# ryantd/tf-operator

Measured on AMD Instinct MI355X. Metric: samples/sec (1-worker TFJob), higher is better.
Workload: dtype bf16

## Files before the change

### csrc/asm/gemm_gen.py

```python
#!/usr/bin/env python3
from __future__ import annotations

import sys

LINE = 1056
HALF = 32 * LINE
STAGE = 2 * HALF
LDS_BYTES = 2 * STAGE
KARG_BYTES = 96

KARG = {
    "X": 0, "W": 8, "C": 16, "S": 24,
    "ldx": 32, "ldw": 36, "ldc": 40, "lds": 44,
    "ktiles": 48, "tiles_m": 52, "tiles_n": 56, "xq": 60, "xr": 64,
    "per_group": 68, "fw": 72, "fc": 76, "map": 80, "grid": 84, "phase": 88, "m": 92,
}
MAP_WALK_COLS = 16
MAP_DEFAULT = 2

EPIS = ("plain", "swiglu_fwd", "swiglu_bwd", "rope", "delta", "resadd")

S_ARGS = 4
S_X, S_W, S_C, S_S = 4, 6, 8, 10
S_LDX, S_LDW, S_LDC, S_LDS = 12, 13, 14, 15
# ... 1846 lines not shown
        parts.append(body)
        metas.append(meta)
    for vname, knobs in SWIGLU_BWD_VARIANTS:
        body, meta = _with_knobs(knobs, lambda: kernel("swiglu_bwd", variant=vname))
        parts.append(body)
        metas.append(meta)
    for epi, vname, knobs in SWIGLU_PERSIST_VARIANTS:
        body, meta = _with_knobs(knobs, lambda: kernel(epi, variant=vname))
        parts.append(body)
        metas.append(meta)
    import attn_gen
    import wgrad_gen

    def wgrad_round4():
        saved = dict(wgrad_gen.KNOBS)
        wgrad_gen.KNOBS.update(map="spread", zero_late=False)
        try:
            return wgrad_gen.kernel("v1")
        finally:
            wgrad_gen.KNOBS.clear()
            wgrad_gen.KNOBS.update(saved)

    import attn_bwd_gen

    for body, meta in (wgrad_gen.kernel(), wgrad_round4(), *attn_gen.all_kernels(), probe_kernel(), kernel("plain", trace=True),
                       _with_knobs({"timing": 1}, lambda: kernel("plain", variant="timing")),
                       _with_knobs({"timing": 2}, lambda: kernel("plain", variant="timing2")),
                       *attn_bwd_gen.all_kernels(),
                       *(kernel_nn(epi) for epi in NN_EPIS)):
        parts.append(body)
        metas.append(meta)
    parts.append(".text\n.p2alignl 6, 3212836864\n.fill 256, 4, 3212836864")
    parts.append(".amdgpu_metadata\n---\namdhsa.version:\n  - 1\n  - 2\namdhsa.target: amdgcn-amd-amdhsa--gfx950\namdhsa.kernels:\n" + "".join(metas)
                 + "...\n.end_amdgpu_metadata")
    return "\n".join(parts) + "\n"


if __name__ == "__main__":
    out = sys.argv[1] if len(sys.argv) > 1 else "gemm_tn_asm.s"
    with open(out, "w") as f:
        f.write(generate())
```

### csrc/hip/attention.hip

```cpp
#include <cstdlib>
#include <cstring>

#include "toa_common.h"

typedef __attribute__((ext_vector_type(8))) short bf16x8;
typedef __attribute__((ext_vector_type(4))) short bf16x4;
typedef __attribute__((ext_vector_type(16))) float f32x16;

#define LOG2E 1.4426950408889634f
#define EXP2(x) __builtin_amdgcn_exp2f(x)
#define RESCALE_THR 8.0f

__device__ __forceinline__ f32x16 mfma32(bf16x8 a, bf16x8 b, f32x16 c) {
  return __builtin_amdgcn_mfma_f32_32x32x16_bf16(a, b, c, 0, 0, 0);
}

__device__ __forceinline__ bf16x8 as_bf16x8(u32x4 v) { return __builtin_bit_cast(bf16x8, v); }

#define TK 64
template <int D>
struct AG {
  static constexpr int NCH = D / 8;
  static constexpr int ROWB = 2 * D;
  static constexpr int NS = D / 16;
// ... 1437 lines not shown
    const char* e = getenv("TOA_ATTN_DKDV");
    return !(e && strcmp(e, "hip") == 0);
  }();
  return g_dkdv_variant == 1 || (g_dkdv_variant < 0 && env_on);
}

template <int D, bool ROPE>
static void dkdv_ds_launch(hipStream_t stream, const bf16_t* q, const bf16_t* k, const bf16_t* v, const bf16_t* dout,
                           const float* nlse2, const float* delta, bf16_t* dk, bf16_t* dv, bf16_t* ds, int B, int H,
                           int Hk, int S, float scale, int o_bshd, const float* cosv, const float* sinv, int H3) {
  if (D == 128 && !g_attn_tstat && attn_dkdv_asm_on()) {
    if (toa_attn_dkdv_asm(q, k, v, dout, nlse2, delta, dk, dv, ds, B, H, Hk, S, D, scale, o_bshd | (ROPE ? 2 : 0),
                          cosv, sinv, H3, stream) == 0)
      return;
  }
  const dim3 grid((S / 128) * B * Hk), block(512);
  if (g_attn_tstat)
    hipLaunchKernelGGL((attn_bwd_dkdv_ds_kernel<D, ROPE, true>), grid, block, 0, stream, q, k, v, dout, nlse2, delta,
                       dk, dv, ds, B, H, Hk, S, scale, scale * LOG2E, o_bshd, cosv, sinv, H3, g_attn_tstat);
  else
    hipLaunchKernelGGL((attn_bwd_dkdv_ds_kernel<D, ROPE>), grid, block, 0, stream, q, k, v, dout, nlse2, delta, dk,
                       dv, ds, B, H, Hk, S, scale, scale * LOG2E, o_bshd, cosv, sinv, H3, nullptr);
}
static bool attn_bwd_uses_ds(int S) { return attn_bwd_variant() >= 1 && S % FWD_QB == 0; }
static int64_t attn_ds_blocks_bytes(int B, int H, int S) {
  const int64_t nb = S / 32;
  return (int64_t)B * H * (nb * (nb + 1) / 2) * 2048;
}
static int64_t attn_ds_bytes(int B, int H, int S) {
  return attn_ds_blocks_bytes(B, H, S) + (int64_t)B * H * S * 4 + 2048;
}
extern "C" int64_t toa_attn_bwd_ws_bytes(int B, int H, int S, int D) {
  (void)D;
  return attn_bwd_uses_ds(S) ? attn_ds_bytes(B, H, S) : 0;
}

template <int D, bool TAIL>
static void attn_set_lds_limits() {
  static bool done = false;
  if (done) return;
  (void)hipFuncSetAttribute((const void*)attn_fwd_kernel<D, TAIL>, hipFuncAttributeMaxDynamicSharedMemorySize,
                            4 * AG<D>::TILEB);
  (void)hipFuncSetAttribute((const void*)attn_bwd_dkdv_kernel<D, TAIL>, hipFuncAttributeMaxDynamicSharedMemorySize,
                            DKV<D>::LDS);
  (void)hipFuncSetAttribute((const void*)attn_bwd_dq_kernel<D, TAIL>, hipFuncAttributeMaxDynamicSharedMemorySize,
                            4 * AG<D>::TILEB);
// ... 20 lines not shown
      return (int)hipGetLastError();
    }
  }
  hipLaunchKernelGGL((attn_fwd_kernel<D, TAIL>), dim3(nqb * H * B), dim3(64 * FWD_WAVES), 4 * AG<D>::TILEB, stream, q, k, v,
                     o, lse, B, H, Hk, S, scale * LOG2E, o_bshd);
  return (int)hipGetLastError();
}

template <int D, bool TAIL>
static int attn_bwd_launch(const bf16_t* q, const bf16_t* k, const bf16_t* v, const bf16_t* o, const bf16_t* dout,
                           const float* lse, float* delta, void* ws, bf16_t* dq, bf16_t* dk, bf16_t* dv, int B, int H,
                           int Hk, int S, int o_bshd, float scale, hipStream_t stream) {
  attn_set_lds_limits<D, TAIL>();
  if constexpr (!TAIL) {
    if (attn_bwd_uses_ds(S)) {
      if (ws == nullptr) return (int)hipErrorInvalidValue;
      bf16_t* ds = (bf16_t*)ws;
      float* nlse2 = (float*)((char*)ws + attn_ds_blocks_bytes(B, H, S));
      const int rows = B * H * S;
      hipLaunchKernelGGL((attn_delta_kernel<D>), dim3((rows + 256 / (D / 8) - 1) / (256 / (D / 8))), dim3(256), 0,
                         stream, o, dout, lse, delta, nlse2, rows, H, S, o_bshd);
      dkdv_ds_launch<D, false>(stream, q, k, v, dout, nlse2, delta, dk, dv, ds, B, H, Hk, S, scale, o_bshd, nullptr,
                               nullptr, 0);
      hipLaunchKernelGGL((attn_bwd_dqg_kernel<D>), dim3((S / FWD_QB) * H * B), dim3(512), 0, stream, k, ds, dq, B, H,
                         Hk, S, scale, nullptr, nullptr, 0);
      return (int)hipGetLastError();
    }
  }
  hipLaunchKernelGGL((attn_bwd_dq_kernel<D, TAIL>), dim3(((S + FWD_QB - 1) / FWD_QB) * H * B), dim3(64 * FWD_WAVES),
                     4 * AG<D>::TILEB, stream, q, k, v, dout, o, lse, delta, dq, B, H, Hk, S, scale, scale * LOG2E,
                     o_bshd);
  hipLaunchKernelGGL((attn_bwd_dkdv_kernel<D, TAIL>), dim3(((S + 127) / 128) * B * Hk), dim3(512), DKV<D>::LDS, stream,
                     q, k, v, dout, lse, delta, dk, dv, B, H, Hk, S, scale, scale * LOG2E, o_bshd);
  return (int)hipGetLastError();
}

static bool attn_shape_ok(int B, int H, int Hk, int S, int D, int flags) {
  return (D == 64 || D == 128) && B > 0 && S > 0 && Hk > 0 && H % Hk == 0 && (flags & 1);
}

extern "C" int toa_attn_fwd_asm(const bf16_t* q, const bf16_t* k, const bf16_t* v, bf16_t* o, float* lse, int B,
                                int H, int Hk, int S, int D, int flags, float scale, hipStream_t stream);
static bool attn_fwd_asm_on() {
  static const bool env_on = [] {
    const char* e = getenv("TOA_ATTN_FWD");
    return !(e && strcmp(e, "hip") == 0);
  }();
  return g_fwd_variant == 2 || (g_fwd_variant < 0 && env_on);
// ... 44 lines not shown
}

extern "C" int toa_attn_bwd_rope(const bf16_t* q, const bf16_t* k, const bf16_t* v, const bf16_t* o,
                                 const bf16_t* dout, const float* lse, float* delta, void* ws, const float* cosv,
                                 const float* sinv, bf16_t* dqkv, int B, int H, int Hk, int S, int D, int flags,
                                 float scale, hipStream_t stream) {
  if (!attn_shape_ok(B, H, Hk, S, D, flags)) return (int)hipErrorInvalidValue;
  if (!attn_bwd_uses_ds(S)) return (int)hipErrorNotSupported;
  if (ws == nullptr || dqkv == nullptr || cosv == nullptr || sinv == nullptr) return (int)hipErrorInvalidValue;
  const int o_bshd = (flags >> 1) & 1;
  const int H3 = H + 2 * Hk;
  bf16_t* ds = (bf16_t*)ws;
  float* nlse2 = (float*)((char*)ws + attn_ds_blocks_bytes(B, H, S));
  const int rows = B * H * S;
#define TOA_ATTN_BWD_ROPE(DD)                                                                                    \
  do {                                                                                                           \
    if (flags & 4)                                                                                               \
      hipLaunchKernelGGL(attn_nlse2_kernel, dim3((rows + 255) / 256), dim3(256), 0, stream, lse, nlse2, rows);   \
    else                                                                                                         \
      hipLaunchKernelGGL((attn_delta_kernel<DD>), dim3((rows + 256 / (DD / 8) - 1) / (256 / (DD / 8))),          \
                         dim3(256), 0, stream, o, dout, lse, delta, nlse2, rows, H, S, o_bshd);                  \
    dkdv_ds_launch<DD, true>(stream, q, k, v, dout, nlse2, delta, dqkv, dqkv, ds, B, H, Hk, S, scale, o_bshd,  \
                             cosv, sinv, H3);                                                                   \
    hipLaunchKernelGGL((attn_bwd_dqg_kernel<DD, true>), dim3((S / FWD_QB) * H * B), dim3(512), 0, stream, k, ds, \
                       dqkv, B, H, Hk, S, scale, cosv, sinv, H3);                                               \
  } while (0)
#ifdef TOA_ATTN_D128_ONLY
  if (D != 128) return (int)hipErrorInvalidValue;
  TOA_ATTN_BWD_ROPE(128);
#else
  if (D == 128)
    TOA_ATTN_BWD_ROPE(128);
  else
    TOA_ATTN_BWD_ROPE(64);
#endif
#undef TOA_ATTN_BWD_ROPE
  return (int)hipGetLastError();
}
```

### csrc/hip/gemm_asm.hip

```cpp
#include <hip/hip_runtime.h>

#include <cstdint>
#include <cstdlib>
#include <cstring>
#include <mutex>

#include "toa_common.h"

namespace {

#include "toa_asm_blob.inc"

constexpr int kMaxDev = 64;
enum { K_PLAIN = 0, K_SWIGLU_FWD = 1, K_SWIGLU_BWD = 2, K_PROBE = 3, K_TRACE = 4, K_TIMING = 5, K_TIMING2 = 6,
       K_WGRAD = 7, K_V1 = 8, K_WGRAD_V1 = 16, K_ATTN_FWD = 17, K_ATTN_D1 = 18, K_ATTN_T1 = 23,
       K_ATTN_DKDV = 26, K_DKDV_D1 = 27, K_DKDV_T1 = 34, K_SWIGLU_FWD_R4 = 41, K_SWIGLU_BWD_R4 = 42, K_SWBWD_V1 = 43, K_PLAIN_V9 = 48, K_DKDV_S7 = 49, K_DKDV_D8 = 50, K_DKDV_S8 = 51, K_SWFWD_P1 = 52, K_SWBWD_P1 = 53, K_ROPE = 54, K_DELTA = 55, K_RESADD = 56, K_N = 57 };
const char* kNames[K_N] = {"toa_gemm_tn_asm_plain",    "toa_gemm_tn_asm_swiglu_fwd", "toa_gemm_tn_asm_swiglu_bwd",
                           "toa_gemm_tn_asm_probe",    "toa_gemm_tn_asm_trace",      "toa_gemm_tn_asm_timing",
                           "toa_gemm_tn_asm_timing2",  "toa_wgrad_nt_asm",           "toa_gemm_tn_asm_plain_v1",
                           "toa_gemm_tn_asm_plain_v2", "toa_gemm_tn_asm_plain_v3", "toa_gemm_tn_asm_plain_v4",
                           "toa_gemm_tn_asm_plain_v5", "toa_gemm_tn_asm_plain_v6", "toa_gemm_tn_asm_plain_v7",
                           "toa_gemm_tn_asm_plain_v8", "toa_wgrad_nt_asm_v1",       "toa_attn_fwd_asm",
                           "toa_attn_fwd_asm_d1",      "toa_attn_fwd_asm_d2",        "toa_attn_fwd_asm_d3",
                           "toa_attn_fwd_asm_d4",      "toa_attn_fwd_asm_d5",        "toa_attn_fwd_asm_t1",
                           "toa_attn_fwd_asm_c1",      "toa_attn_fwd_asm_t2",        "toa_attn_dkdv_asm",
                           "toa_attn_dkdv_asm_d1",     "toa_attn_dkdv_asm_d2",       "toa_attn_dkdv_asm_d3",
                           "toa_attn_dkdv_asm_d4",     "toa_attn_dkdv_asm_d5",       "toa_attn_dkdv_asm_d6",
                           "toa_attn_dkdv_asm_d7",     "toa_attn_dkdv_asm_t1",
                           "toa_attn_dkdv_asm_s1",     "toa_attn_dkdv_asm_s2",       "toa_attn_dkdv_asm_s3",
                           "toa_attn_dkdv_asm_s4",     "toa_attn_dkdv_asm_s5",       "toa_attn_dkdv_asm_s6",
                           "toa_gemm_tn_asm_swiglu_fwd_r4", "toa_gemm_tn_asm_swiglu_bwd_r4",
                           "toa_gemm_tn_asm_swiglu_bwd_b1", "toa_gemm_tn_asm_swiglu_bwd_b2",
                           "toa_gemm_tn_asm_swiglu_bwd_b3", "toa_gemm_tn_asm_swiglu_bwd_b4",
                           "toa_gemm_tn_asm_swiglu_bwd_b5",
                           "toa_gemm_tn_asm_plain_v9",
                           "toa_attn_dkdv_asm_s7", "toa_attn_dkdv_asm_d8", "toa_attn_dkdv_asm_s8",
                           "toa_gemm_tn_asm_swiglu_fwd_p1", "toa_gemm_tn_asm_swiglu_bwd_p1",
                           "toa_gemm_tn_asm_rope",
                           "toa_gemm_tn_asm_delta",
                           "toa_gemm_tn_asm_resadd"};

enum { NN_PLAIN = 0, NN_SWIGLU_BWD = 1, NN_DELTA = 2, NN_N = 3 };
const char* kNnNames[NN_N] = {"toa_gemm_nn_asm_plain", "toa_gemm_nn_asm_swiglu_bwd", "toa_gemm_nn_asm_delta"};

constexpr int kNnBase = 1 << 16;

struct DevModule {
  std::once_flag once;
  hipError_t err = hipSuccess;
  hipModule_t mod = nullptr;
  hipFunction_t fn[K_N] = {};
  hipFunction_t nn[NN_N] = {};
};
DevModule g_mod[kMaxDev];

hipFunction_t get_fn(int which, hipError_t* err) {
  int dev = 0;
  if ((*err = hipGetDevice(&dev)) != hipSuccess) return nullptr;
  if (dev < 0 || dev >= kMaxDev) {
    *err = hipErrorInvalidDevice;
    return nullptr;
  }
  DevModule& m = g_mod[dev];
  std::call_once(m.once, [&m]() {
    m.err = hipModuleLoadData(&m.mod, toa_asm_blob);
    for (int i = 0; m.err == hipSuccess && i < K_N; ++i) m.err = hipModuleGetFunction(&m.fn[i], m.mod, kNames[i]);
    for (int i = 0; m.err == hipSuccess && i < NN_N; ++i) m.err = hipModuleGetFunction(&m.nn[i], m.mod, kNnNames[i]);
  });
  *err = m.err;
  return m.err == hipSuccess ? (which >= kNnBase ? m.nn[which - kNnBase] : m.fn[which]) : nullptr;
}

struct __attribute__((packed)) Args {
  uint64_t X, W, C, S;
  uint32_t ldx, ldw, ldc, lds;
  uint32_t ktiles, tiles_m, tiles_n, xq, xr, per_group;
  uint32_t fw, fc;
  uint32_t map;
  uint32_t grid;
  uint32_t phase;
  uint32_t m;
};
static_assert(sizeof(Args) == 96, "kernarg block must match csrc/asm/gemm_gen.py KARG_BYTES");

constexpr uint32_t kMapDefault = 2;
constexpr uint32_t kMapWalkCols = 16;

bool ld_ok(int64_t ld, int64_t min_cols) { return ld >= min_cols && ld % 8 == 0 && ld * 2 * 256 < (1ll << 32); }
bool al16(const void* p) { return ((uintptr_t)p & 15) == 0; }

constexpr int kNumPlainVariants = 9;
constexpr int kVariantFn[kNumPlainVariants] = {K_V1,     K_V1 + 1, K_V1 + 2, K_V1 + 3,  K_V1 + 4,
                                               K_V1 + 5, K_V1 + 6, K_V1 + 7, K_PLAIN_V9};
// ... 612 lines not shown
  a.dout = (uint64_t)dout;
  a.nlse2 = (uint64_t)nlse2;
  a.ndelta = (uint64_t)ndelta;
  a.dk = (uint64_t)dk;
  a.dv = (uint64_t)dv;
  a.ds = (uint64_t)ds;
  a.cosv = (uint64_t)cosv;
  a.sinv = (uint64_t)sinv;
  a.B = (uint32_t)B;
  a.H = (uint32_t)H;
  a.Hk = (uint32_t)Hk;
  a.S = (uint32_t)S;
  a.scale = scale;
  a.c = scale * 1.4426950408889634f;
  a.flags = (uint32_t)flags;
  a.rep = (uint32_t)(H / Hk);
  a.nkb = (uint32_t)(S / 128);
  a.H3 = (uint32_t)(rope ? H3 : 0);
  a.dbg = (uint64_t)dbg;
  size_t sz = sizeof(a);
  void* cfg[] = {HIP_LAUNCH_PARAM_BUFFER_POINTER, &a, HIP_LAUNCH_PARAM_BUFFER_SIZE, &sz, HIP_LAUNCH_PARAM_END};
  return (int)hipModuleLaunchKernel(fn, (unsigned)nwg, 1, 1, 256, 1, 1, 0, stream, nullptr, cfg);
}
```

### tf_operator_amd/ops/_lib.py

```python
from __future__ import annotations

import ctypes
import os
import threading

import torch

_HERE = os.path.dirname(os.path.abspath(__file__))
LIB_PATH = os.environ.get("TOA_HIP_LIB") or os.path.join(os.path.dirname(_HERE), "lib", "libtoa_hip.so")

_lock = threading.Lock()
_lib = None
_err = None

c_int = ctypes.c_int
c_i64 = ctypes.c_int64
c_f = ctypes.c_float
c_p = ctypes.c_void_p

_SIGS = {
    "toa_sumsq": [c_p, c_i64, c_int, c_p, c_p, c_int, c_p],
    "toa_adamw_flat": [c_p, c_p, c_p, c_int, c_p, c_p, c_i64, c_f, c_f, c_f, c_f, c_f, c_int, c_f, c_p, c_f, c_p],
    "toa_adamw_flat_dstep": [c_p, c_p, c_p, c_int, c_p, c_p, c_i64, c_f, c_f, c_f, c_f, c_f, c_p, c_f, c_p, c_f,
                             c_p],
# ... 74 lines not shown
    "toa_gemm_asm_rows": [c_p, c_i64, c_p, c_i64, c_p, c_i64, c_int, c_int, c_int, c_p],
    "toa_gemm_asm_swiglu": [c_p, c_i64, c_p, c_i64, c_p, c_i64, c_p, c_i64, c_int, c_int, c_int, c_p],
    "toa_gemm_asm_swiglu_bwd": [c_p, c_i64, c_p, c_i64, c_p, c_i64, c_p, c_i64, c_int, c_int, c_int, c_p],
    "toa_gemm_asm_swiglu_bwd_variant": [c_int, c_p, c_i64, c_p, c_i64, c_p, c_i64, c_p, c_i64, c_int, c_int, c_int, c_p],
    "toa_gemm_asm_available": [],
    "toa_gemm_asm_trace": [c_p, c_p, c_i64, c_p, c_i64, c_p, c_i64, c_int, c_int, c_int, c_p],
    "toa_host_free": [c_p],
    "toa_gemm_asm_stage": [c_int, c_p, c_i64, c_p, c_i64, c_p, c_i64, c_int, c_int, c_int, c_p],
    "toa_gemm_asm_variant": [c_int, c_p, c_i64, c_p, c_i64, c_p, c_i64, c_int, c_int, c_int, c_p],
    "toa_gemm_asm_map": [c_int, c_p, c_i64, c_p, c_i64, c_p, c_i64, c_int, c_int, c_int, c_p],
    "toa_gemm_asm_set_epi_variant": [c_int],
    "toa_gemm_asm_set_phase": [c_int, ctypes.c_uint],
    "toa_wgrad_asm_set_map": [c_int],
    "toa_gemm_asm_set_map": [c_int],
    "toa_gemm_asm_set_persist": [c_int],
    "toa_attn_dkdv_asm_set_arm": [c_int],
    "toa_gemm_asm_timing": [c_int, c_p, c_p, c_i64, c_p, c_i64, c_p, c_i64, c_int, c_int, c_int, c_p],
    "toa_gemm_asm_probe": [c_p, c_p, c_i64, c_p, c_i64, c_p, c_i64, c_int, c_int, c_int, c_p],
    "toa_attn_set_bwd_variant": [c_int],
    "toa_attn_set_bwd_timing": [c_p],
    "toa_norm_set_row": [c_int],
    "toa_attn_set_fwd_variant": [c_int],
    "toa_attn_set_dkdv_variant": [c_int],
    "toa_attn_dkdv_asm": [c_p, c_p, c_p, c_p, c_p, c_p, c_p, c_p, c_p, c_int, c_int, c_int, c_int, c_int, c_f, c_int,
                          c_p, c_p, c_int, c_p],
    "toa_attn_dkdv_asm_variant": [c_int, c_p, c_p, c_p, c_p, c_p, c_p, c_p, c_p, c_p, c_int, c_int, c_int, c_int, c_int,
                                  c_f, c_int, c_p, c_p, c_int, c_p],
    "toa_attn_dkdv_asm_timing": [c_p, c_p, c_p, c_p, c_p, c_p, c_p, c_p, c_p, c_p, c_int, c_int, c_int, c_int, c_int,
                                 c_f, c_int, c_p, c_p, c_int, c_p],
    "toa_attn_bwd_rope": [c_p, c_p, c_p, c_p, c_p, c_p, c_p, c_p, c_p, c_p, c_p, c_int, c_int, c_int, c_int, c_int,
                          c_int, c_f, c_p],
    "toa_emulate_xfer": [c_p, c_p, c_i64, c_int, ctypes.c_double, c_p],
    "toa_emulate_copy_nocu": [c_p, c_p, c_i64, c_p],
    "toa_flag_publish": [c_p, ctypes.c_uint, c_p],
    "toa_flags_wait": [c_p, c_int, c_int, c_int, ctypes.c_uint, c_p, c_int, c_p],
    "toa_copy_nocu": [c_p, c_p, c_i64, c_p],
    "toa_sum_slices_bf16": [c_p, c_p, c_int, c_i64, c_i64, c_p],
    "toa_gemm_tune": [c_int, c_int, c_i64, c_i64, c_i64, c_p, c_i64, c_p, c_i64, c_p, c_i64, c_f, c_int, c_p, c_p, c_p,
                      c_p, c_p, c_int],
    "toa_gemm_kernel_name": [c_int, c_int, c_i64, c_i64, c_i64, c_i64, c_i64, c_i64, c_int, c_int, c_p, c_int],
}


def _load():
    global _lib, _err
    with _lock:
# ... 101 lines not shown
```

Baseline: 6.583.

## Add hand-written assembly kernel for attention backward dQ from stored dS

```diff
diff --git a/csrc/asm/attn_dq_gen.py b/csrc/asm/attn_dq_gen.py
--- /dev/null
+++ b/csrc/asm/attn_dq_gen.py
@@ -0,0 +1,508 @@
+#!/usr/bin/env python3
+from __future__ import annotations
+
+import sys
+
+import attn_gen as AG
+import gemm_gen as G
+from attn_gen import Item, schedule
+from gemm_gen import Asm, ar, sr, vr
+
+NAME = "toa_attn_dq_asm"
+D = 128
+ROWB = 2 * D
+TK = 64
+KT = TK * ROWB
+DSB = 2048
+DSW = 4 * DSB
+SLOT = KT + 4 * DSW
+NSLOT = 3
+LDS_BYTES = NSLOT * SLOT
+RING = 6
+LEAD = 4
+DL_DMA = 10
+KARG_BYTES = 80
+KARG = {"K": 0, "dS": 8, "dQ": 16, "cos": 24, "sin": 32, "B": 40, "H": 44, "Hk": 48, "S": 52, "scale": 56,
+        "flags": 60, "nqb": 64, "rep": 68, "g8": 72, "H3": 76}
+
+S_K, S_DS, S_DQP, S_COS, S_SIN = 4, 6, 8, 10, 12
+S_B, S_H, S_HK, S_S, S_SC, S_FL = 14, 15, 16, 17, 18, 19
+S_NQB, S_REP, S_G8, S_H3 = 20, 21, 22, 23
+S_W, S_QB, S_HH, S_BB, S_HKV = 24, 25, 26, 27, 28
+S_T, S_TW, S_TL = 29, 30, 31
+S_CUR, S_NX, S_IT, S_NXK, S_NXD, S_KSO, S_DSA0, S_DSA1 = 32, 33, 34, 35, 36, 37, 38, 39
+SRD_K, SRD_DS, SRD_O, SRD_C, SRD_S = 40, 44, 48, 52, 56
+S_T0 = AG.S_T0
+S_DQ, S_DR = AG.S_DQ, AG.S_DR
+S_TRI0, S_TRI1, S_KM0, S_DM0, S_Q0, S_OSTR, S_SOFF, S_OJ = 70, 71, 72, 73, 74, 75, 76, 77
+N_SGPR = 96
+assert (S_T0, S_DQ, S_DR) == (60, 68, 69)
+
+V_TRO, V_TRO8, V_DSO = 1, 5, 9
+V_CTRO, V_CTRO8, V_CDSO = 13, 17, 21
+V_T = 24
+V_KD = 32
+V_DSG = 36
+V_KF = 40
+V_SF = 64
+V_CS, V_SN = 96, 160
+V_X = 224
+A_ACC = 0
+
+
+def kf(f):
+    return V_KF + 4 * (f % RING)
+
+
+def sfreg(j, n, s2):
+    return V_SF + 4 * (4 * j + 2 * n + s2)
+
+
+def k_piece(u: int) -> list[str]:
+    return [f"s_add_u32 m0, {sr(S_NXK)}, {1024 * u}",
+            "s_nop 0",
+            f"buffer_load_dwordx4 {vr(V_KD + u)}, {sr(SRD_K, 4)}, {sr(S_KSO)} offen lds"]
+
+
+def ds_piece(j: int, n: int, half: int) -> list[str]:
+    base = S_DSA0 if j == 0 else S_DSA1
+    out = [f"s_add_u32 {sr(S_SOFF)}, {sr(base)}, {DSB}"] if n else []
+    so = S_SOFF if n else base
+    return out + [f"s_add_u32 m0, {sr(S_NXD)}, {2 * DSB * j + DSB * n + 1024 * half}",
+                  "s_nop 0",
+                  f"buffer_load_dwordx4 {vr(V_DSG + half)}, {sr(SRD_DS, 4)}, {sr(so)} offen nt lds"]
+
+
+def dma_setup() -> list[str]:
+    return [f"s_lshl_b32 {sr(S_KSO)}, {sr(S_IT)}, 14",
+            f"s_add_u32 {sr(S_NXK)}, {sr(S_NX)}, {sr(S_KM0)}",
+            f"s_lshl_b32 {sr(S_T0)}, {sr(S_IT)}, 12",
+            f"s_add_u32 {sr(S_DSA0)}, {sr(S_TRI0)}, {sr(S_T0)}",
+            f"s_add_u32 {sr(S_DSA1)}, {sr(S_TRI1)}, {sr(S_T0)}",
+            f"s_add_u32 {sr(S_NXD)}, {sr(S_NX)}, {sr(S_DM0)}"]
+
+
+N_FULL, N_DIAG, N_KONLY = 12, 10, 4
+
+
+def issue_generic(a: Asm):
+    skip, nods = a.fresh("iss_done"), a.fresh("iss_no01")
+    a(f"s_cmp_gt_u32 {sr(S_IT)}, {sr(S_TL)}")
+    a(f"s_cbranch_scc1 {skip}")
+    for x in dma_setup():
+        a(x)
+    for u in range(4):
+        for x in k_piece(u):
+            a(x)
+    a(f"s_cmp_gt_u32 {sr(S_IT)}, {sr(S_TW)}")
+    a(f"s_cbranch_scc1 {skip}")
+    for half in range(2):
+        for x in ds_piece(0, 0, half):
+            a(x)
+    a(f"s_cmp_eq_u32 {sr(S_IT)}, {sr(S_TW)}")
+    a(f"s_cbranch_scc1 {nods}")
+    for half in range(2):
+        for x in ds_piece(0, 1, half):
+            a(x)
+    a.label(nods)
+    for n in range(2):
+        for half in range(2):
+            for x in ds_piece(1, n, half):
+                a(x)
+    a.label(skip)
+
+
+def tile_mfmas(diag: bool) -> list:
+    out = []
+    for n in range(2):
+        for s2 in range(2):
+            for dt in range(4):
+                f = 8 * n + 4 * s2 + dt
+                for j in range(2):
+                    if diag and n == 1 and j == 0:
+                        continue
+                    acc = ar(A_ACC + 64 * j + 16 * dt, 16)
+                    out.append((f"v_mfma_f32_32x32x16_bf16 {acc}, {vr(kf(f), 4)}, {vr(sfreg(j, n, s2), 4)}, {acc}",
+                                [f"KF{f}", f"SF{j}{n}{s2}"]))
+    return out
+
+
+def kt_read(f: int) -> list[str]:
+    n, r = divmod(f, 8)
+    s2, dt = divmod(r, 4)
+    rb = (32 * n + 16 * s2) * ROWB
+    return [f"ds_read_b64_tr_b16 {vr(kf(f), 2)}, {vr(V_CTRO + dt)} offset:{rb} ; KF{f}",
+            f"ds_read_b64_tr_b16 {vr(kf(f) + 2, 2)}, {vr(V_CTRO8 + dt)} offset:{rb} ; KF{f}"]
+
+
+def ds_read(j: int, n: int, s2: int) -> list[str]:
+    off = 2 * DSB * j + DSB * n
+    return [f"ds_read_b64_tr_b16 {vr(sfreg(j, n, s2), 2)}, {vr(V_CDSO + 2 * s2)} offset:{off} ; SF{j}{n}{s2}",
+            f"ds_read_b64_tr_b16 {vr(sfreg(j, n, s2) + 2, 2)}, {vr(V_CDSO + 2 * s2 + 1)} offset:{off} ; SF{j}{n}{s2}"]
+
+
+def slot_offsets(a: Asm):
+    for i in range(4):
+        a(f"v_add_u32 {vr(V_CTRO + i)}, {sr(S_CUR)}, {vr(V_TRO + i)}")
+        a(f"v_add_u32 {vr(V_CTRO8 + i)}, {sr(S_CUR)}, {vr(V_TRO8 + i)}")
+        a(f"v_add_u32 {vr(V_CDSO + i)}, {sr(S_CUR)}, {vr(V_DSO + i)}")
+
+
+def compute(a: Asm, diag: bool, dma: bool, tail: list | None = None):
+    mf = tile_mfmas(diag)
+    first: dict = {}
+    last: dict = {}
+    for g, (_, tags) in enumerate(mf):
+        for t in tags:
+            first.setdefault(t, g)
+            last[t] = g
+    items: list[Item] = []
+    for f in range(16):
+        rel = -1 if f < RING else last[f"KF{f - RING}"]
+        items.append(Item(kt_read(f), 8, rel, max(rel, first[f"KF{f}"] - LEAD), "kr"))
+    for n in range(2):
+        for s2 in range(2):
+            for j in range(2):
+                if diag and n == 1 and j == 0:
+                    continue
+                items.append(Item(ds_read(j, n, s2), 8, -1, max(-1, first[f"SF{j}{n}{s2}"] - LEAD), "sr"))
+    if dma:
+        for u in range(4):
+            items.append(Item(k_piece(u), 48, -1, DL_DMA, "dma", split=False))
+        for j in range(2):
+            for n in range(2):
+                for half in range(2):
+                    items.append(Item(ds_piece(j, n, half), 48, -1, DL_DMA, "dma", split=False))
+    slot_offsets(a)
+    schedule(a, mf, items, tail)
+
+
+def coords(a: Asm):
+    t0, t1 = S_T0, S_T0 + 1
+    a(f"s_cmp_eq_u32 {sr(S_NQB)}, 0")
+    a(f"s_cbranch_scc1 {a.abort}")
+    a(f"s_lshl_b32 {sr(t0)}, {sr(S_NQB)}, 8")
+    a(f"s_cmp_lg_u32 {sr(t0)}, {sr(S_S)}")
+    a(f"s_cbranch_scc1 {a.abort}")
+    a(f"s_mul_i32 {sr(t0)}, {sr(S_REP)}, {sr(S_HK)}")
+    a(f"s_cmp_lg_u32 {sr(t0)}, {sr(S_H)}")
+    a(f"s_cbranch_scc1 {a.abort}")
+    a(f"s_mul_i32 {sr(t0)}, {sr(S_NQB)}, {sr(S_H)}")
+    a(f"s_mul_i32 {sr(t0)}, {sr(t0)}, {sr(S_B)}")
+    a(f"s_cmp_ge_u32 s2, {sr(t0)}")
+    a(f"s_cbranch_scc1 {a.abort}")
+    a(f"s_mul_i32 {sr(t1)}, {sr(S_B)}, {sr(S_HK)}")
+    lgen, lcoord = a.fresh("coords_generic"), a.fresh("coords_done")
+    a(f"s_cmp_eq_u32 {sr(S_G8)}, 0")
+    a(f"s_cbranch_scc1 {lgen}")
+    a(f"s_and_b32 {sr(t0 + 2)}, {sr(t1)}, 7")
+    a(f"s_cmp_lg_u32 {sr(t0 + 2)}, 0")
+    a(f"s_cbranch_scc1 {a.abort}")
+    a(f"s_and_b32 {sr(S_T0 + 2)}, s2, 7")
+    a(f"s_lshr_b32 {sr(S_T0 + 3)}, s2, 3")
+    a(f"s_lshr_b32 {sr(S_T0 + 4)}, {sr(t1)}, 3")
+    a(f"s_mul_i32 {sr(S_T0 + 5)}, {sr(S_T0 + 4)}, {sr(S_REP)}")
+    AG.udiv(a, S_DQ, S_DR, S_T0 + 3, S_T0 + 5)
+    a(f"s_sub_u32 {sr(S_QB)}, {sr(S_NQB)}, 1")
+    a(f"s_sub_u32 {sr(S_QB)}, {sr(S_QB)}, {sr(S_DQ)}")
+    a(f"s_mov_b32 {sr(S_T0 + 3)}, {sr(S_DR)}")
+    AG.udiv(a, S_DQ, S_DR, S_T0 + 3, S_REP)
+    a(f"s_mul_i32 {sr(S_T0 + 2)}, {sr(S_T0 + 2)}, {sr(S_T0 + 4)}")
+    a(f"s_add_u32 {sr(S_T0 + 2)}, {sr(S_T0 + 2)}, {sr(S_DQ)}")
+    a(f"s_mov_b32 {sr(S_T0 + 5)}, {sr(S_DR)}")
+    AG.udiv(a, S_DQ, S_DR, S_T0 + 2, S_HK)
+    a(f"s_mov_b32 {sr(S_BB)}, {sr(S_DQ)}")
+    a(f"s_mul_i32 {sr(S_HH)}, {sr(S_DR)}, {sr(S_REP)}")
+    a(f"s_add_u32 {sr(S_HH)}, {sr(S_HH)}, {sr(S_T0 + 5)}")
+    a(f"s_branch {lcoord}")
+    a.label(lgen)
+    a(f"s_mul_i32 {sr(S_T0 + 2)}, {sr(S_H)}, {sr(S_B)}")
+    AG.udiv(a, S_DQ, S_DR, 2, S_T0 + 2)
+    a(f"s_sub_u32 {sr(S_QB)}, {sr(S_NQB)}, 1")
+    a(f"s_sub_u32 {sr(S_QB)}, {sr(S_QB)}, {sr(S_DQ)}")
+    a(f"s_mov_b32 {sr(S_T0 + 3)}, {sr(S_DR)}")
+    AG.udiv(a, S_DQ, S_DR, S_T0 + 3, S_H)
+    a(f"s_mov_b32 {sr(S_BB)}, {sr(S_DQ)}")
+    a(f"s_mov_b32 {sr(S_HH)}, {sr(S_DR)}")
+    a.label(lcoord)
+    AG.udiv(a, S_DQ, S_DR, S_HH, S_REP)
+    a(f"s_mov_b32 {sr(S_HKV)}, {sr(S_DQ)}")
+
+
+def prologue(a: Asm):
+    a(f"s_load_dwordx16 {sr(4, 16)}, s[0:1], 0x0")
+    a(f"s_load_dwordx4 {sr(20, 4)}, s[0:1], 0x40")
+    a(f"v_lshrrev_b32 {vr(V_X + 15)}, 6, v0")
+    a("s_waitcnt lgkmcnt(0)")
+    coords(a)
+    t0, t1, t2 = S_T0, S_T0 + 1, S_T0 + 2
+    a("s_nop 4")
+    a(f"v_readfirstlane_b32 {sr(S_W)}, {vr(V_X + 15)}")
+    a("s_nop 4")
+    a(f"s_lshl_b32 {sr(t0)}, {sr(S_QB)}, 2")
+    a(f"s_add_u32 {sr(S_TL)}, {sr(t0)}, 3")
+    a(f"s_add_u32 {sr(S_TW)}, {sr(t0)}, {sr(S_W)}")
+    a(f"s_lshl_b32 {sr(S_Q0)}, {sr(S_QB)}, 8")
+    a(f"s_lshl_b32 {sr(t0)}, {sr(S_W)}, 6")
+    a(f"s_add_u32 {sr(S_Q0)}, {sr(S_Q0)}, {sr(t0)}")
+    a(f"s_lshl_b32 {sr(t0)}, {sr(S_TW)}, 1")
+    a(f"s_add_u32 {sr(t1)}, {sr(t0)}, 1")
+    a(f"s_mul_i32 {sr(t0)}, {sr(t0)}, {sr(t1)}")
+    a(f"s_lshr_b32 {sr(t0)}, {sr(t0)}, 1")
+    a(f"s_lshl_b32 {sr(S_TRI0)}, {sr(t0)}, 11")
+    a(f"s_lshl_b32 {sr(t1)}, {sr(t1)}, 11")
+    a(f"s_add_u32 {sr(S_TRI1)}, {sr(S_TRI0)}, {sr(t1)}")
+    a(f"s_lshl_b32 {sr(S_KM0)}, {sr(S_W)}, 12")
+    a(f"s_lshl_b32 {sr(S_DM0)}, {sr(S_W)}, 13")
+    a(f"s_add_u32 {sr(S_DM0)}, {sr(S_DM0)}, {KT}")
+    a(f"s_mul_i32 {sr(t1)}, {sr(S_BB)}, {sr(S_HK)}")
+    a(f"s_add_u32 {sr(t1)}, {sr(t1)}, {sr(S_HKV)}")
+    a(f"s_mul_i32 {sr(t1)}, {sr(t1)}, {sr(S_S)}")
+    a(f"s_lshl_b32 {sr(t2)}, {sr(S_S)}, 8")
+    AG.srd64(a, SRD_K, S_K, t1, ROWB, sr(t2))
+    a(f"s_lshr_b32 {sr(t0)}, {sr(S_S)}, 5")
+    a(f"s_add_u32 {sr(t1)}, {sr(t0)}, 1")
+    a(f"s_mul_i32 {sr(t0)}, {sr(t0)}, {sr(t1)}")
+    a(f"s_lshr_b32 {sr(t0)}, {sr(t0)}, 1")
+    a(f"s_lshl_b32 {sr(t2)}, {sr(t0)}, 11")
+    a(f"s_mul_i32 {sr(t1)}, {sr(S_BB)}, {sr(S_H)}")
+    a(f"s_add_u32 {sr(t1)}, {sr(t1)}, {sr(S_HH)}")
+    AG.srd64(a, SRD_DS, S_DS, t1, sr(t2), sr(t2))
+    lrope, lodone = a.fresh("o_rope"), a.fresh("o_done")
+    a(f"s_bitcmp1_b32 {sr(S_FL)}, 0")
+    a(f"s_cbranch_scc1 {lrope}")
+    a(f"s_mul_i32 {sr(t1)}, {sr(t1)}, {sr(S_S)}")
+    a(f"s_add_u32 {sr(t1)}, {sr(t1)}, {sr(S_Q0)}")
+    a(f"s_mov_b32 {sr(S_OSTR)}, {ROWB}")
+    AG.srd64(a, SRD_O, S_DQP, t1, ROWB, 64 * ROWB)
+    a(f"s_branch {lodone}")
+    a.label(lrope)
+    a(f"s_mul_i32 {sr(t1)}, {sr(S_BB)}, {sr(S_S)}")
+    a(f"s_add_u32 {sr(t1)}, {sr(t1)}, {sr(S_Q0)}")
+    a(f"s_mul_i32 {sr(t1)}, {sr(t1)}, {sr(S_H3)}")
+    a(f"s_add_u32 {sr(t1)}, {sr(t1)}, {sr(S_HH)}")
+    a(f"s_lshl_b32 {sr(S_OSTR)}, {sr(S_H3)}, 8")
+    a(f"s_mul_i32 {sr(t2)}, {sr(S_OSTR)}, 63")
+    a(f"s_add_u32 {sr(t2)}, {sr(t2)}, {ROWB}")
+    AG.srd64(a, SRD_O, S_DQP, t1, ROWB, sr(t2))
+    AG.srd64(a, SRD_C, S_COS, S_Q0, 256, 64 * 256)
+    AG.srd64(a, SRD_S, S_SIN, S_Q0, 256, 64 * 256)
+    a.label(lodone)
+    l, g, qq, pp, hh, r, tt = (V_X + i for i in range(7))
+    t = V_T
+    a(f"v_and_b32 {vr(l)}, 63, v0")
+    a(f"v_lshrrev_b32 {vr(g)}, 4, {vr(l)}")
+    a(f"v_bfe_u32 {vr(qq)}, {vr(l)}, 2, 2")
+    a(f"v_and_b32 {vr(pp)}, 3, {vr(l)}")
+    a(f"v_lshrrev_b32 {vr(hh)}, 5, {vr(l)}")
+    a(f"v_and_b32 {vr(r)}, 31, {vr(l)}")
+    a(f"v_lshl_add_u32 {vr(tt)}, {vr(hh)}, 2, {vr(qq)}")
+    a(f"v_lshlrev_b32 {vr(tt)}, 8, {vr(tt)}")
+    a(f"v_and_b32 {vr(t)}, 1, {vr(g)}")
+    a(f"v_lshlrev_b32 {vr(t)}, 1, {vr(t)}")
+    a(f"v_lshrrev_b32 {vr(t + 1)}, 1, {vr(pp)}")
+    a(f"v_add_u32 {vr(t)}, {vr(t)}, {vr(t + 1)}")
+    a(f"v_lshl_add_u32 {vr(t + 1)}, {vr(qq)}, 2, {vr(hh)}")
+    a(f"v_add_u32 {vr(t + 2)}, 2, {vr(t + 1)}")
+    a(f"v_and_b32 {vr(t + 3)}, 1, {vr(pp)}")
+    a(f"v_lshlrev_b32 {vr(t + 3)}, 3, {vr(t + 3)}")
+    a(f"v_add_u32 {vr(t + 6)}, {vr(t + 3)}, {vr(tt)}")
+    for dt in range(4):
+        a(f"v_add_u32 {vr(t + 4)}, {4 * dt}, {vr(t)}")
+        a(f"v_xor_b32 {vr(t + 5)}, {vr(t + 4)}, {vr(t + 1)}")
+        a(f"v_lshl_add_u32 {vr(V_TRO + dt)}, {vr(t + 5)}, 4, {vr(t + 6)}")
+        a(f"v_xor_b32 {vr(t + 5)}, {vr(t + 4)}, {vr(t + 2)}")
+        a(f"v_lshl_add_u32 {vr(V_TRO8 + dt)}, {vr(t + 5)}, 4, {vr(t + 6)}")
+        a(f"v_add_u32 {vr(V_TRO8 + dt)}, {8 * ROWB}, {vr(V_TRO8 + dt)}")
+    a(f"v_lshl_add_u32 {vr(t + 4)}, {vr(t)}, 2, {vr(qq)}")
+    a(f"v_lshl_add_u32 {vr(t + 4)}, {vr(hh)}, 2, {vr(t + 4)}")
+    a(f"v_lshlrev_b32 {vr(t + 5)}, 9, {vr(t)}")
+    a(f"v_add_u32 {vr(t + 5)}, {vr(t + 5)}, {vr(t + 3)}")
+    a(f"v_add_u32 {vr(t + 5)}, {sr(S_DM0)}, {vr(t + 5)}")
+    for s2 in range(2):
+        for e in range(2):
+            a(f"v_add_u32 {vr(t + 7)}, {16 * s2 + 8 * e}, {vr(t + 4)}")
+            a(f"v_and_b32 {vr(t + 7)}, 31, {vr(t + 7)}")
+            a(f"v_lshl_add_u32 {vr(V_DSO + 2 * s2 + e)}, {vr(t + 7)}, 4, {vr(t + 5)}")
+    a(f"v_and_b32 {vr(t)}, 15, {vr(l)}")
+    a(f"v_lshlrev_b32 {vr(t + 1)}, 2, {vr(g)}")
+    a(f"v_xor_b32 {vr(t)}, {vr(t)}, {vr(t + 1)}")
+    a(f"v_lshlrev_b32 {vr(t + 1)}, 8, {vr(g)}")
+    a(f"v_add_u32 {vr(t + 1)}, {sr(S_KM0)}, {vr(t + 1)}")
+    for u in range(4):
+        a(f"v_xor_b32 {vr(t + 2)}, {u}, {vr(t)}")
+        a(f"v_lshl_add_u32 {vr(V_KD + u)}, {vr(t + 2)}, 4, {vr(t + 1)}")
+        a(f"v_add_u32 {vr(V_KD + u)}, {4 * u * ROWB}, {vr(V_KD + u)}")
+    for half in range(2):
+        a(f"v_add_u32 {vr(t)}, {2 * half}, {vr(hh)}")
+        a(f"v_lshlrev_b32 {vr(t + 1)}, 2, {vr(t)}")
+        a(f"v_sub_u32 {vr(t + 1)}, {vr(r)}, {vr(t + 1)}")
+        a(f"v_and_b32 {vr(t + 1)}, 31, {vr(t + 1)}")
+        a(f"v_lshl_add_u32 {vr(t + 1)}, {vr(t)}, 5, {vr(t + 1)}")
+        a(f"v_lshlrev_b32 {vr(V_DSG + half)}, 4, {vr(t + 1)}")
+    lnr = a.fresh("no_rope_rows")
+    a(f"s_bitcmp1_b32 {sr(S_FL)}, 0")
+    a(f"s_cbranch_scc0 {lnr}")
+    a(f"v_lshlrev_b32 {vr(t)}, 8, {vr(r)}")
+    a(f"v_lshl_add_u32 {vr(t)}, {vr(hh)}, 4, {vr(t)}")
+    a(f"s_mov_b32 {sr(S_OJ)}, {32 * 256}")
+    for j in range(2):
+        so = sr(S_OJ) if j else "0"
+        for dt in range(2):
+            for g4 in range(4):
+                o = 128 * dt + 32 * g4
+                a(f"buffer_load_dwordx4 {vr(V_CS + 32 * j + 16 * dt + 4 * g4, 4)}, {vr(t)}, {sr(SRD_C, 4)}, {so} "
+                  f"offen offset:{o}")
+                a(f"buffer_load_dwordx4 {vr(V_SN + 32 * j + 16 * dt + 4 * g4, 4)}, {vr(t)}, {sr(SRD_S, 4)}, {so} "
+                  f"offen offset:{o}")
+    a.label(lnr)
+    for x in range(128):
+        a(f"v_accvgpr_write_b32 {ar(A_ACC + x)}, 0")
+    for tile in range(2):
+        a(f"s_mov_b32 {sr(S_IT)}, {tile}")
+        a(f"s_mov_b32 {sr(S_NX)}, {tile * SLOT}")
+        issue_generic(a)
+    a(f"s_mov_b32 {sr(S_T)}, 0")
+    a(f"s_mov_b32 {sr(S_CUR)}, 0")
+    a(f"s_mov_b32 {sr(S_NX)}, {2 * SLOT}")
+
+
+def store_rows(a: Asm, j: int, scaled: bool):
+    oo = V_X + 2
+    so = sr(S_OJ) if j else "0"
+    for dt in range(4):
+        for k in range(2):
+            tmp, data = V_X + 4, V_X + 12
+            base = A_ACC + 64 * j + 16 * dt + 8 * k
+            for e in range(8):
+                a(f"v_accvgpr_read_b32 {vr(tmp + e)}, {ar(base + e)}")
+            if scaled:
+                for e in range(8):
+                    a(f"v_mul_f32 {vr(tmp + e)}, {sr(S_SC)}, {vr(tmp + e)}")
+            for e in range(4):
+                a(f"v_cvt_pk_bf16_f32 {vr(data + e)}, {vr(tmp + 2 * e)}, {vr(tmp + 2 * e + 1)}")
+            a("s_nop 1")
+            a(f"v_permlane32_swap_b32 {vr(data)}, {vr(data + 2)}")
+            a(f"v_permlane32_swap_b32 {vr(data + 1)}, {vr(data + 3)}")
+            a(f"buffer_store_dwordx4 {vr(data, 4)}, {vr(oo)}, {sr(SRD_O, 4)}, {so} offen offset:{64 * dt + 32 * k}")
+            a("s_nop 1")
+
+
+def epilogue(a: Asm):
+    a("s_waitcnt vmcnt(0)")
+    a("s_nop 7")
+    a("s_nop 7")
+    a("s_nop 7")
+    r, hh, oo = V_X, V_X + 1, V_X + 2
+    a(f"v_and_b32 {vr(r)}, 31, v0")
+    a(f"v_bfe_u32 {vr(hh)}, v0, 5, 1")
+    a(f"v_mul_lo_u32 {vr(oo)}, {vr(r)}, {sr(S_OSTR)}")
+    a(f"v_lshl_add_u32 {vr(oo)}, {vr(hh)}, 4, {vr(oo)}")
+    a(f"s_lshl_b32 {sr(S_OJ)}, {sr(S_OSTR)}, 5")
+    lrope, ldone = a.fresh("epi_rope"), a.fresh("epi_done")
+    a(f"s_bitcmp1_b32 {sr(S_FL)}, 0")
+    a(f"s_cbranch_scc1 {lrope}")
+    for j in range(2):
+        store_rows(a, j, True)
+    a(f"s_branch {ldone}")
+    a.label(lrope)
+    y1, y2, p, q = V_T, V_T + 1, V_T + 2, V_T + 3
+    for j in range(2):
+        for dt in range(2):
+            for i in range(16):
+                a1, a2 = A_ACC + 64 * j + 16 * dt + i, A_ACC + 64 * j + 16 * (dt + 2) + i
+                c, s_ = V_CS + 32 * j + 16 * dt + i, V_SN + 32 * j + 16 * dt + i
+                a(f"v_accvgpr_read_b32 {vr(y1)}, {ar(a1)}")
+                a(f"v_accvgpr_read_b32 {vr(y2)}, {ar(a2)}")
+                a(f"v_mul_f32 {vr(y1)}, {sr(S_SC)}, {vr(y1)}")
+                a(f"v_mul_f32 {vr(y2)}, {sr(S_SC)}, {vr(y2)}")
+                a(f"v_mul_f32 {vr(p)}, {vr(s_)}, {vr(y2)}")
+                a(f"v_mul_f32 {vr(q)}, {vr(s_)}, {vr(y1)}")
+                a(f"v_fma_f32 {vr(p)}, {vr(c)}, {vr(y1)}, {vr(p)}")
+                a(f"v_fma_f32 {vr(q)}, {vr(c)}, {vr(y2)}, -{vr(q)}")
+                a(f"v_accvgpr_write_b32 {ar(a1)}, {vr(p)}")
+                a(f"v_accvgpr_write_b32 {ar(a2)}, {vr(q)}")
+    a("s_nop 1")
+    for j in range(2):
+        store_rows(a, j, False)
+    a.label(ldone)
+
+
+def kernel() -> tuple[str, str]:
+    a = Asm(prefix="dq_")
+    a.raw(f".globl {NAME}")
+    a.raw(".p2align 8")
+    a.raw(f".type {NAME},@function")
+    a.raw(f"{NAME}:")
+    prologue(a)
+    lab = {k: a.fresh(k) for k in ("loop", "steady", "next", "w10", "w4", "w0", "wd", "nocomp", "diag", "epi")}
+    t1, t2 = S_T0 + 1, S_T0 + 2
+    a.label(lab["loop"])
+    a(f"s_add_u32 {sr(S_IT)}, {sr(S_T)}, 2")
+    a(f"s_cmp_lt_u32 {sr(S_IT)}, {sr(S_TW)}")
+    a(f"s_cbranch_scc1 {lab['steady']}")
+    a(f"s_add_u32 {sr(t1)}, {sr(S_T)}, 1")
+    a(f"s_cmp_gt_u32 {sr(t1)}, {sr(S_TL)}")
+    a(f"s_cbranch_scc1 {lab['w0']}")
+    a(f"s_cmp_gt_u32 {sr(t1)}, {sr(S_TW)}")
+    a(f"s_cbranch_scc1 {lab['w4']}")
+    a(f"s_cmp_eq_u32 {sr(t1)}, {sr(S_TW)}")
+    a(f"s_cbranch_scc1 {lab['w10']}")
+    a(f"s_waitcnt vmcnt({N_FULL})")
+    a(f"s_branch {lab['wd']}")
+    a.label(lab["w10"])
+    a(f"s_waitcnt vmcnt({N_DIAG})")
+    a(f"s_branch {lab['wd']}")
+    a.label(lab["w4"])
+    a(f"s_waitcnt vmcnt({N_KONLY})")
+    a(f"s_branch {lab['wd']}")
+    a.label(lab["w0"])
+    a("s_waitcnt vmcnt(0)")
+    a.label(lab["wd"])
+    a("s_barrier")
+    issue_generic(a)
+    a(f"s_cmp_gt_u32 {sr(S_T)}, {sr(S_TW)}")
+    a(f"s_cbranch_scc1 {lab['next']}")
+    a(f"s_cmp_eq_u32 {sr(S_T)}, {sr(S_TW)}")
+    a(f"s_cbranch_scc1 {lab['diag']}")
+    compute(a, False, False, [f"s_branch {lab['next']}"])
+    a.label(lab["diag"])
+    compute(a, True, False, [f"s_branch {lab['next']}"])
+    a.label(lab["steady"])
+    a(f"s_waitcnt vmcnt({N_FULL})")
+    a("s_barrier")
+    for x in dma_setup():
+        a(x)
+    compute(a, False, True)
+    a.label(lab["next"])
+    a(f"s_mov_b32 {sr(S_NX)}, {sr(S_CUR)}")
+    a(f"s_add_u32 {sr(S_CUR)}, {sr(S_CUR)}, {SLOT}")
+    a(f"s_cmp_eq_u32 {sr(S_CUR)}, {NSLOT * SLOT}")
+    a(f"s_cselect_b32 {sr(S_CUR)}, 0, {sr(S_CUR)}")
+    a(f"s_add_u32 {sr(S_T)}, {sr(S_T)}, 1")
+    a(f"s_cmp_gt_u32 {sr(S_T)}, {sr(S_TL)}")
+    a(f"s_cbranch_scc0 {lab['loop']}")
+    epilogue(a)
+    a.label(a.abort)
+    a("s_waitcnt vmcnt(0)")
+    a("s_endpgm")
+    a.raw(f".size {NAME}, .-{NAME}")
+    desc, meta = G._descriptor(NAME, lds_bytes=LDS_BYTES, n_sgpr=N_SGPR, karg_bytes=KARG_BYTES)
+    return "\n".join(a.out) + "\n" + desc, meta
+
+
+def all_kernels() -> list[tuple[str, str]]:
+    return [kernel()]
+
+
+def generate(kernels=None) -> str:
+    kernels = kernels or [kernel()]
+    return "\n".join(['.amdgcn_target "amdgcn-amd-amdhsa--gfx950"', ".amdhsa_code_object_version 5", ".text",
+                      *(b for b, _ in kernels),
+                      ".amdgpu_metadata\n---\namdhsa.version:\n  - 1\n  - 2\namdhsa.target: amdgcn-amd-amdhsa--gfx950\n"
+                      "amdhsa.kernels:\n" + "".join(m for _, m in kernels) + "...\n.end_amdgpu_metadata"]) + "\n"
+
+
+if __name__ == "__main__":
+    with open(sys.argv[1] if len(sys.argv) > 1 else "attn_dq_asm.s", "w") as f:
+        f.write(generate())
diff --git a/csrc/asm/gemm_gen.py b/csrc/asm/gemm_gen.py
--- a/csrc/asm/gemm_gen.py
+++ b/csrc/asm/gemm_gen.py
@@ -1892,12 +1892,14 @@
             wgrad_gen.KNOBS.update(saved)
 
     import attn_bwd_gen
+    import attn_dq_gen
 
     for body, meta in (wgrad_gen.kernel(), wgrad_round4(), *attn_gen.all_kernels(), probe_kernel(), kernel("plain", trace=True),
                        _with_knobs({"timing": 1}, lambda: kernel("plain", variant="timing")),
                        _with_knobs({"timing": 2}, lambda: kernel("plain", variant="timing2")),
                        *attn_bwd_gen.all_kernels(),
-                       *(kernel_nn(epi) for epi in NN_EPIS)):
+                       *(kernel_nn(epi) for epi in NN_EPIS),
+                       *attn_dq_gen.all_kernels()):
         parts.append(body)
         metas.append(meta)
     parts.append(".text\n.p2alignl 6, 3212836864\n.fill 256, 4, 3212836864")
diff --git a/csrc/hip/attention.hip b/csrc/hip/attention.hip
--- a/csrc/hip/attention.hip
+++ b/csrc/hip/attention.hip
@@ -1483,6 +1483,35 @@
     hipLaunchKernelGGL((attn_bwd_dkdv_ds_kernel<D, ROPE>), grid, block, 0, stream, q, k, v, dout, nlse2, delta, dk,
                        dv, ds, B, H, Hk, S, scale, scale * LOG2E, o_bshd, cosv, sinv, H3, nullptr);
 }
+extern "C" int toa_attn_dq_asm(const bf16_t* k, const bf16_t* ds, bf16_t* dq, int B, int H, int Hk, int S, int D,
+                               float scale, int flags, const float* cosv, const float* sinv, int H3,
+                               hipStream_t stream);
+static int g_dq_variant = -1;
+extern "C" int toa_attn_set_dq_variant(int v) {
+  if (v < -1 || v > 1) return (int)hipErrorInvalidValue;
+  g_dq_variant = v;
+  return 0;
+}
+static constexpr bool kAttnDqAsmDefault = true;
+static bool attn_dq_asm_on() {
+  static const bool env_on = [] {
+    const char* e = getenv("TOA_ATTN_DQ");
+    if (e && strcmp(e, "hip") == 0) return false;
+    if (e && strcmp(e, "asm") == 0) return true;
+    return kAttnDqAsmDefault;
+  }();
+  return g_dq_variant == 1 || (g_dq_variant < 0 && env_on);
+}
+
+template <int D, bool ROPE>
+static void dq_ds_launch(hipStream_t stream, const bf16_t* k, const bf16_t* ds, bf16_t* dq, int B, int H, int Hk,
+                         int S, float scale, const float* cosv, const float* sinv, int H3) {
+  if (D == 128 && attn_dq_asm_on()) {
+    if (toa_attn_dq_asm(k, ds, dq, B, H, Hk, S, D, scale, ROPE ? 1 : 0, cosv, sinv, H3, stream) == 0) return;
+  }
+  hipLaunchKernelGGL((attn_bwd_dqg_kernel<D, ROPE>), dim3((S / FWD_QB) * H * B), dim3(512), 0, stream, k, ds, dq, B,
+                     H, Hk, S, scale, cosv, sinv, H3);
+}
 static bool attn_bwd_uses_ds(int S) { return attn_bwd_variant() >= 1 && S % FWD_QB == 0; }
 static int64_t attn_ds_blocks_bytes(int B, int H, int S) {
   const int64_t nb = S / 32;
@@ -1549,8 +1578,7 @@
                          stream, o, dout, lse, delta, nlse2, rows, H, S, o_bshd);
       dkdv_ds_launch<D, false>(stream, q, k, v, dout, nlse2, delta, dk, dv, ds, B, H, Hk, S, scale, o_bshd, nullptr,
                                nullptr, 0);
-      hipLaunchKernelGGL((attn_bwd_dqg_kernel<D>), dim3((S / FWD_QB) * H * B), dim3(512), 0, stream, k, ds, dq, B, H,
-                         Hk, S, scale, nullptr, nullptr, 0);
+      dq_ds_launch<D, false>(stream, k, ds, dq, B, H, Hk, S, scale, nullptr, nullptr, 0);
       return (int)hipGetLastError();
     }
   }
@@ -1641,8 +1669,7 @@
                          dim3(256), 0, stream, o, dout, lse, delta, nlse2, rows, H, S, o_bshd);                  \
     dkdv_ds_launch<DD, true>(stream, q, k, v, dout, nlse2, delta, dqkv, dqkv, ds, B, H, Hk, S, scale, o_bshd,  \
                              cosv, sinv, H3);                                                                   \
-    hipLaunchKernelGGL((attn_bwd_dqg_kernel<DD, true>), dim3((S / FWD_QB) * H * B), dim3(512), 0, stream, k, ds, \
-                       dqkv, B, H, Hk, S, scale, cosv, sinv, H3);                                               \
+    dq_ds_launch<DD, true>(stream, k, ds, dqkv, B, H, Hk, S, scale, cosv, sinv, H3);                            \
   } while (0)
 #ifdef TOA_ATTN_D128_ONLY
   if (D != 128) return (int)hipErrorInvalidValue;
diff --git a/csrc/hip/gemm_asm.hip b/csrc/hip/gemm_asm.hip
--- a/csrc/hip/gemm_asm.hip
+++ b/csrc/hip/gemm_asm.hip
@@ -45,12 +45,17 @@
 
 constexpr int kNnBase = 1 << 16;
 
+enum { DQ_ATTN = 0, DQ_N = 1 };
+const char* kDqNames[DQ_N] = {"toa_attn_dq_asm"};
+constexpr int kDqBase = 2 << 16;
+
 struct DevModule {
   std::once_flag once;
   hipError_t err = hipSuccess;
   hipModule_t mod = nullptr;
   hipFunction_t fn[K_N] = {};
   hipFunction_t nn[NN_N] = {};
+  hipFunction_t dq[DQ_N] = {};
 };
 DevModule g_mod[kMaxDev];
 
@@ -66,9 +71,12 @@
     m.err = hipModuleLoadData(&m.mod, toa_asm_blob);
     for (int i = 0; m.err == hipSuccess && i < K_N; ++i) m.err = hipModuleGetFunction(&m.fn[i], m.mod, kNames[i]);
     for (int i = 0; m.err == hipSuccess && i < NN_N; ++i) m.err = hipModuleGetFunction(&m.nn[i], m.mod, kNnNames[i]);
+    for (int i = 0; m.err == hipSuccess && i < DQ_N; ++i) m.err = hipModuleGetFunction(&m.dq[i], m.mod, kDqNames[i]);
   });
   *err = m.err;
-  return m.err == hipSuccess ? (which >= kNnBase ? m.nn[which - kNnBase] : m.fn[which]) : nullptr;
+  if (m.err != hipSuccess) return nullptr;
+  if (which >= kDqBase) return m.dq[which - kDqBase];
+  return which >= kNnBase ? m.nn[which - kNnBase] : m.fn[which];
 }
 
 struct __attribute__((packed)) Args {
@@ -727,3 +735,49 @@
   void* cfg[] = {HIP_LAUNCH_PARAM_BUFFER_POINTER, &a, HIP_LAUNCH_PARAM_BUFFER_SIZE, &sz, HIP_LAUNCH_PARAM_END};
   return (int)hipModuleLaunchKernel(fn, (unsigned)nwg, 1, 1, 256, 1, 1, 0, stream, nullptr, cfg);
 }
+
+struct __attribute__((packed)) DqArgs {
+  uint64_t k, ds, dq, cosv, sinv;
+  uint32_t B, H, Hk, S;
+  float scale;
+  uint32_t flags, nqb, rep, g8, H3;
+};
+static_assert(sizeof(DqArgs) == 80, "kernarg block must match csrc/asm/attn_dq_gen.py KARG_BYTES");
+
+extern "C" int toa_attn_dq_asm(const bf16_t* k, const bf16_t* ds, bf16_t* dq, int B, int H, int Hk, int S, int D,
+                               float scale, int flags, const float* cosv, const float* sinv, int H3,
+                               hipStream_t stream) {
+  const bool rope = (flags & 1) != 0;
+  if (D != 128 || B <= 0 || H <= 0 || Hk <= 0 || H % Hk || S <= 0 || S % 256 || !al16(k) || !al16(ds) || !al16(dq) ||
+      (flags & ~1) || (rope && (!cosv || !sinv || !al16(cosv) || !al16(sinv) || H3 != H + 2 * Hk)))
+    return (int)hipErrorInvalidValue;
+  const int64_t nb = S / 32, nblk = nb * (nb + 1) / 2;
+  const int64_t nwg = (int64_t)(S / 256) * H * B;
+  if (nwg >= (1 << 24) || nblk * 2048 >= (1ll << 32) || (int64_t)S * 256 >= (1ll << 31) ||
+      (int64_t)B * H * S >= (1ll << 32) || (int64_t)B * S * (rope ? H3 : 1) >= (1ll << 32) ||
+      (int64_t)64 * (rope ? H3 : 1) * 256 >= (1ll << 31))
+    return (int)hipErrorInvalidValue;
+  hipError_t err;
+  hipFunction_t fn = get_fn(kDqBase + DQ_ATTN, &err);
+  if (!fn) return (int)err;
+  DqArgs a;
+  memset(&a, 0, sizeof(a));
+  a.k = (uint64_t)k;
+  a.ds = (uint64_t)ds;
+  a.dq = (uint64_t)dq;
+  a.cosv = (uint64_t)cosv;
+  a.sinv = (uint64_t)sinv;
+  a.B = (uint32_t)B;
+  a.H = (uint32_t)H;
+  a.Hk = (uint32_t)Hk;
+  a.S = (uint32_t)S;
+  a.scale = scale;
+  a.flags = (uint32_t)flags;
+  a.nqb = (uint32_t)(S / 256);
+  a.rep = (uint32_t)(H / Hk);
+  a.g8 = ((int64_t)B * Hk) % 8 == 0 ? 1u : 0u;
+  a.H3 = (uint32_t)(rope ? H3 : 0);
+  size_t sz = sizeof(a);
+  void* cfg[] = {HIP_LAUNCH_PARAM_BUFFER_POINTER, &a, HIP_LAUNCH_PARAM_BUFFER_SIZE, &sz, HIP_LAUNCH_PARAM_END};
+  return (int)hipModuleLaunchKernel(fn, (unsigned)nwg, 1, 1, 256, 1, 1, 0, stream, nullptr, cfg);
+}
diff --git a/tf_operator_amd/ops/_lib.py b/tf_operator_amd/ops/_lib.py
--- a/tf_operator_amd/ops/_lib.py
+++ b/tf_operator_amd/ops/_lib.py
@@ -120,6 +120,8 @@
     "toa_norm_set_row": [c_int],
     "toa_attn_set_fwd_variant": [c_int],
     "toa_attn_set_dkdv_variant": [c_int],
+    "toa_attn_set_dq_variant": [c_int],
+    "toa_attn_dq_asm": [c_p, c_p, c_p, c_int, c_int, c_int, c_int, c_int, c_f, c_int, c_p, c_p, c_int, c_p],
     "toa_attn_dkdv_asm": [c_p, c_p, c_p, c_p, c_p, c_p, c_p, c_p, c_p, c_int, c_int, c_int, c_int, c_int, c_f, c_int,
                           c_p, c_p, c_int, c_p],
     "toa_attn_dkdv_asm_variant": [c_int, c_p, c_p, c_p, c_p, c_p, c_p, c_p, c_p, c_p, c_int, c_int, c_int, c_int, c_int,
```

Result: no change. 6.593 (median of 4 runs) (+0.2%).
